# cwangrun/MGProto

Hardware: NVIDIA H100
Metric: images/sec (higher is better)
Workload: dtype f32

## Files before the change

mgproto_b200/csrc/abi.cu:

```cuda
#include "mgp_common.cuh"
#include <stdlib.h>
#include <string.h>

int mgp_logprob_simt_launch(const float* xhat, const float* mu, const float* sigma, float eps, float eps_log,
                            float* out, int layout, int B, int HW, int P, int D, float* ws, cudaStream_t st);
bool mgp_logprob_tc_supported(int layout, int B, int HW, int P, int D, int assume_iso);
size_t mgp_logprob_tc_ws_bytes(long long N, int P, int D);
int mgp_logprob_tc_launch(const float* xhat, const float* mu, const float* sigma, float eps, float eps_log,
                          float* out, int layout, int B, int HW, int P, int D, void* ws, size_t ws_bytes,
                          int reuse_operands, int assume_iso, int x_staged, cudaStream_t st);

extern "C" int mgp_abi_version(void) { return MGP_ABI_VERSION; }

extern "C" const char* mgp_error_string(int code) {
    switch (code) {
        case MGP_OK: return "ok";
        case MGP_ERR_INVALID: return "mgproto_b200: invalid argument (null pointer, non-positive size or misalignment)";
        case MGP_ERR_UNSUPPORTED: return "mgproto_b200: shape not supported by the sm_90a kernels";
        case MGP_ERR_WORKSPACE: return "mgproto_b200: workspace too small";
        default: break;
    }
    if (code > 0) return cudaGetErrorString((cudaError_t)code);
    return "mgproto_b200: unknown error";
}

int g_mgp_em_fused = -1;
int mgp_opt_em_fused() {
    if (g_mgp_em_fused < 0) g_mgp_em_fused = getenv("MGP_EM_UNFUSED") ? 0 : 1;
    return g_mgp_em_fused;
}
void mgp_em_tc_set_prof(void* p, int cls);
extern "C" int mgp_debug_set_ptr(const char* key, void* p, int arg) {
    if (!key) return MGP_ERR_INVALID;
#ifdef MGP_WITH_TC
    if (strcmp(key, "em_tc_prof") == 0) { mgp_em_tc_set_prof(p, arg); return MGP_OK; }
#endif
    return MGP_ERR_INVALID;
}
int g_mgp_tc_z = -1;
int mgp_opt_tc_z() {
    if (g_mgp_tc_z < 0) g_mgp_tc_z = getenv("MGP_TC_NO_Z") ? 0 : 1;
    return g_mgp_tc_z;
}
int g_mgp_em_tc = -1;
int mgp_opt_em_tc() {
    if (g_mgp_em_tc < 0) g_mgp_em_tc = getenv("MGP_EM_NO_TC") ? 0 : 1;
    return g_mgp_em_tc;
}
int g_mgp_em_pipe = -1;
int mgp_opt_em_pipe() {
    if (g_mgp_em_pipe < 0) g_mgp_em_pipe = getenv("MGP_EM_NO_PIPE") ? 0 : 1;
    return g_mgp_em_pipe;
}
extern "C" int mgp_set_option(const char* key, int value) {
    if (!key) return MGP_ERR_INVALID;
    if (strcmp(key, "em_pipe") == 0) {
        const int prev = mgp_opt_em_pipe();
        g_mgp_em_pipe = value ? 1 : 0;
        return prev;
    }
    if (strcmp(key, "tc_z") == 0) {
        const int prev = mgp_opt_tc_z();
        g_mgp_tc_z = value ? 1 : 0;
        return prev;
    }
    if (strcmp(key, "em_tc") == 0) {
        const int prev = mgp_opt_em_tc();
        g_mgp_em_tc = value ? 1 : 0;
        return prev;
    }
    if (strcmp(key, "em_fused") == 0) {
        const int prev = mgp_opt_em_fused();
        g_mgp_em_fused = value ? 1 : 0;
        return prev;
    }
    return MGP_ERR_INVALID;
}

extern "C" int mgp_has_tensor_core_path(void) {
#ifdef MGP_WITH_TC
    return 1;
#else
    return 0;
#endif
}

extern "C" size_t mgp_logprob_ws_bytes(int B, int HW, int P, int D, int math) {
    size_t simt = ((size_t)P * D + P) * sizeof(float);
#ifdef MGP_WITH_TC
    if (math != MGP_MATH_FP32 && mgp_logprob_tc_supported(0, B, HW, P, D, math == MGP_MATH_TC_ISO || math == MGP_MATH_TC_ISO_REUSE)) {
        size_t tc = mgp_logprob_tc_ws_bytes((long long)B * HW, P, D);
        return tc > simt ? tc : simt;
    }
#endif
    (void)math; (void)B; (void)HW;
    return simt;
}

bool mgp_logprob_tcz_supported(int P, int D);
extern "C" int mgp_logprob_ws_is_prototype_only(int out_layout, int P, int D, int math) {
#ifdef MGP_WITH_TC
    return (out_layout == MGP_OUT_LOGP_NP && (math == MGP_MATH_TC_ISO || math == MGP_MATH_TC_ISO_REUSE) && mgp_opt_tc_z() &&
            P > 0 && mgp_logprob_tcz_supported(P, D)) ? 1 : 0;
#else
    (void)out_layout; (void)P; (void)D; (void)math;
    return 0;
#endif
}

extern "C" int mgp_logprob_fwd(const float* xhat_nd, const float* mu, const float* sigma, float eps, float eps_log,
                               float* out, int out_layout, int B, int HW, int P, int D, int math, void* ws,
                               size_t ws_bytes, void* stream) {
    const int x_staged = (math & MGP_MATH_X_STAGED_ISO) ? 1 : ((math & MGP_MATH_X_STAGED) ? 2 : 0);
    math &= 0xff;
    if (!xhat_nd || !mu || !sigma || !out || !ws) return MGP_ERR_INVALID;
    if (B <= 0 || HW <= 0 || P <= 0 || D <= 0 || (D & 3)) return MGP_ERR_INVALID;
    if (out_layout < MGP_OUT_LOGP_NP || out_layout > MGP_OUT_TOP1_BP) return MGP_ERR_INVALID;
    if (!mgp_aligned16(xhat_nd) || !mgp_aligned16(mu) || !mgp_aligned16(sigma) || !mgp_aligned16(out) ||
        !mgp_aligned16(ws))
        return MGP_ERR_INVALID;
    if ((long long)B * HW > 0x7fffffffLL) return MGP_ERR_UNSUPPORTED;
    if (ws_bytes < mgp_logprob_ws_bytes(B, HW, P, D, math)) return MGP_ERR_WORKSPACE;
    cudaStream_t st = (cudaStream_t)stream;
#ifdef MGP_WITH_TC
    const bool iso_mode = (math == MGP_MATH_TC_ISO || math == MGP_MATH_TC_ISO_REUSE);
    if (math == MGP_MATH_TC || math == MGP_MATH_AUTO || math == MGP_MATH_TC_REUSE || iso_mode) {
        if (mgp_logprob_tc_supported(out_layout, B, HW, P, D, iso_mode))
            return mgp_logprob_tc_launch(xhat_nd, mu, sigma, eps, eps_log, out, out_layout, B, HW, P, D, ws, ws_bytes,
                                         math == MGP_MATH_TC_REUSE ? 2 : (math == MGP_MATH_TC_ISO_REUSE ? 1 : 0), iso_mode,
                                         x_staged, st);
        if (math != MGP_MATH_AUTO) return MGP_ERR_UNSUPPORTED;
    }
#else
    if (math == MGP_MATH_TC || math == MGP_MATH_TC_REUSE || math == MGP_MATH_TC_ISO || math == MGP_MATH_TC_ISO_REUSE)
        return MGP_ERR_UNSUPPORTED;
#endif
    if (out_layout == MGP_OUT_TOP1_BP) return MGP_ERR_UNSUPPORTED;
    return mgp_logprob_simt_launch(xhat_nd, mu, sigma, eps, eps_log, out, out_layout, B, HW, P, D,
                                   reinterpret_cast<float*>(ws), st);
}
```

mgproto_b200/csrc/head.cu:

```cuda
#include "mgp_common.cuh"
#include <type_traits>

namespace {

template <int R, int NR>
__device__ __forceinline__ void warp_topT(const float* const (&rows)[NR], int rs, int HW, int T, int lane,
                                          float (&out_v)[NR], int (&out_i)[NR]) {
    unsigned key[NR][R];
#pragma unroll
    for (int i = 0; i < NR; ++i) {
#pragma unroll
        for (int r = 0; r < R; ++r) {
            const int j = lane + 32 * r;
            key[i][r] = (j < HW) ? f2key(rows[i][(size_t)j * rs]) : 0u;
        }
        out_v[i] = 0.f;
        out_i[i] = 0;
    }
    for (int t = 0; t < T; ++t) {
#pragma unroll
        for (int i = 0; i < NR; ++i) {
            unsigned lm = key[i][0];
#pragma unroll
            for (int r = 1; r < R; ++r) lm = max(lm, key[i][r]);
// ... 248 lines not shown
        for (int i = threadIdx.x; i < K * D; i += NTHR) same = same && (s_ri[i] == s_ri[(i / D) * D]);
        const bool iso = __syncthreads_and(same ? 1 : 0) != 0;
        for (int k = warp; k < K; k += NTHR / 32) {
            float mm = 0.f;
            for (int d = lane; d < D; d += 32) mm = fmaf(s_mu[k * D + d], s_mu[k * D + d], mm);
            mm = warp_sum(mm);
            if (lane == 0) s_mm[k] = mm;
        }
        __syncthreads();
        const int KHh = (K + 1) / 2;
        for (int it = threadIdx.x; it < 2 * HW; it += NTHR) {
            const int n = it >> 1, kb = (it & 1) * KHh, ke = min(K, kb + KHh);
            const float4* xr = reinterpret_cast<const float4*>(xhat + ((size_t)b * HW + n) * D);
            for (int k0 = kb; k0 < ke; k0 += 5) {
                float q[5] = {0.f, 0.f, 0.f, 0.f, 0.f};
                float2 q2[5], xx2 = make_float2(0.f, 0.f);
#pragma unroll
                for (int i = 0; i < 5; ++i) q2[i] = make_float2(0.f, 0.f);
                for (int d0 = 0; d0 < D / 4; d0 += 8) {
                    float4 xv[8];
#pragma unroll
                    for (int u = 0; u < 8; ++u) xv[u] = (d0 + u < D / 4) ? __ldg(xr + d0 + u) : make_float4(0.f, 0.f, 0.f, 0.f);
                    if (iso) {
#pragma unroll
                        for (int u = 0; u < 8; ++u) {
                            if (d0 + u >= D / 4) break;
                            const float2 x01 = make_float2(xv[u].x, xv[u].y), x23 = make_float2(xv[u].z, xv[u].w);
                            xx2 = ffma2(x01, x01, xx2);
                            xx2 = ffma2(x23, x23, xx2);
#pragma unroll
                            for (int i = 0; i < 5; ++i) {
                                const int k = min(k0 + i, K - 1);
                                const float4 m = *reinterpret_cast<const float4*>(s_mu + k * D + 4 * (d0 + u));
                                q2[i] = ffma2(x01, make_float2(m.x, m.y), q2[i]);
                                q2[i] = ffma2(x23, make_float2(m.z, m.w), q2[i]);
                            }
                        }
                    } else {
#pragma unroll
                        for (int u = 0; u < 8; ++u) {
                            if (d0 + u >= D / 4) break;
#pragma unroll
                            for (int i = 0; i < 5; ++i) {
                                const int k = min(k0 + i, K - 1);
                                const float4 m = *reinterpret_cast<const float4*>(s_mu + k * D + 4 * (d0 + u));
                                const float4 r = *reinterpret_cast<const float4*>(s_ri + k * D + 4 * (d0 + u));
                                float t;
                                t = (xv[u].x - m.x) * r.x; q[i] = fmaf(t, t, q[i]);
                                t = (xv[u].y - m.y) * r.y; q[i] = fmaf(t, t, q[i]);
                                t = (xv[u].z - m.z) * r.z; q[i] = fmaf(t, t, q[i]);
                                t = (xv[u].w - m.w) * r.w; q[i] = fmaf(t, t, q[i]);
                            }
                        }
                    }
                }
                if (iso) {
                    const float xx = xx2.x + xx2.y;
#pragma unroll
                    for (int i = 0; i < 5; ++i) {
                        const int k = min(k0 + i, K - 1);
                        const float ri = s_ri[k * D];
                        q[i] = ri * ri * (xx - 2.0f * (q2[i].x + q2[i].y) + s_mm[k]);
                    }
                }
#pragma unroll
                for (int i = 0; i < 5; ++i)
                    if (k0 + i < ke) lp[(k0 + i) * HWp + n] = -s_ls[k0 + i] - 0.5f * q[i];
            }
        }
        __syncthreads();
        for (int k0 = warp * NR; k0 < K; k0 += (NTHR / 32) * NR) {
            const float* rows[NR];
#pragma unroll
            for (int i = 0; i < NR; ++i) rows[i] = lp + min(k0 + i, K - 1) * HWp;
            float v[NR];
            int ix[NR];
            if (R <= 8) warp_topT_sorted<(R <= 8 ? R : 1), NR>(rows, 1, HW, T, lane, v, ix);
            else warp_topT<R, NR>(rows, 1, HW, T, lane, v, ix);
#pragma unroll
            for (int i = 0; i < NR; ++i) {
                const int k = k0 + i;
                if (k < K && lane < T) {
                    const int p = (int)g * K + k;
                    const float e = expf(v[i]);
                    winT[k * T + lane] = e;
                    vals[((size_t)b * P + p) * T + lane] = e;
                    idx[((size_t)b * P + p) * T + lane] = ix[i];
                }
            }
        }
    }
    __syncthreads();
    for (int e = threadIdx.x; e < C * T; e += NTHR) {
        const int c = e / T, t = e - c * T;
        const bool own = gok && (long long)c == g;
        float s = 0.f;
        for (int k = 0; k < K; ++k) s = fmaf(s_wd[c * K + k], own ? winT[k * T + t] : win0[c * K + k], s);
        logits[((size_t)b * C + c) * T + t] = logf(s);
    }
}

__global__ void proto_weight_kernel(const float* __restrict__ mu, const float* __restrict__ sigma,
                                    float* __restrict__ w, float* __restrict__ wm, float* __restrict__ wsc,
                                    int* __restrict__ noniso, size_t n, int D) {
    size_t i = (size_t)blockIdx.x * blockDim.x + threadIdx.x;
    if (i < n) {
        const float s = sigma[i];
        const float ww = 1.0f / (s * s);
        w[i] = ww;
        wm[i] = ww * mu[i];
        const size_t p = i / D;
        if (i == p * D) wsc[p] = ww;
        if (s != sigma[p * D]) atomicOr(noniso, 1);
    }
}

constexpr int LCAP = 2304;

template <int VEC> struct LaneVec { float v[VEC]; };
template <int VEC>
__device__ __forceinline__ LaneVec<VEC> lv_ldg(const float* p) {
    LaneVec<VEC> r;
    if constexpr (VEC == 4) { const float4 t = __ldg(reinterpret_cast<const float4*>(p)); r.v[0] = t.x; r.v[1] = t.y; r.v[2] = t.z; r.v[3] = t.w; }
    else { const float2 t = __ldg(reinterpret_cast<const float2*>(p)); r.v[0] = t.x; r.v[1] = t.y; }
    return r;
}
template <int VEC>
__device__ __forceinline__ LaneVec<VEC> lv_ldcg(const float* p) {
    LaneVec<VEC> r;
    if constexpr (VEC == 4) { const float4 t = __ldcg(reinterpret_cast<const float4*>(p)); r.v[0] = t.x; r.v[1] = t.y; r.v[2] = t.z; r.v[3] = t.w; }
    else { const float2 t = __ldcg(reinterpret_cast<const float2*>(p)); r.v[0] = t.x; r.v[1] = t.y; }
    return r;
}
template <int VEC>
__device__ __forceinline__ LaneVec<VEC> lv_ld(const float* p) {
    LaneVec<VEC> r;
    if constexpr (VEC == 4) { const float4 t = *reinterpret_cast<const float4*>(p); r.v[0] = t.x; r.v[1] = t.y; r.v[2] = t.z; r.v[3] = t.w; }
    else { const float2 t = *reinterpret_cast<const float2*>(p); r.v[0] = t.x; r.v[1] = t.y; }
    return r;
}
template <int VEC>
__device__ __forceinline__ void lv_st(float* p, const LaneVec<VEC>& r) {
    if constexpr (VEC == 4) *reinterpret_cast<float4*>(p) = make_float4(r.v[0], r.v[1], r.v[2], r.v[3]);
    else *reinterpret_cast<float2*>(p) = make_float2(r.v[0], r.v[1]);
}
template <int VEC>
__device__ __forceinline__ LaneVec<VEC> lv_zero() {
    LaneVec<VEC> r;
#pragma unroll
    for (int i = 0; i < VEC; ++i) r.v[i] = 0.f;
    return r;
}

template <int VEC>
__global__ void __launch_bounds__(256, VEC == 4 ? 2 : 4)
head_bwd_kernel(const float* __restrict__ gl, const float* __restrict__ logits, const float* __restrict__ vals,
                const int32_t* __restrict__ idx, const float* __restrict__ weight, const int64_t* __restrict__ gt,
                const float* __restrict__ xhat, const float* __restrict__ w, const float* __restrict__ wm,
                const float* __restrict__ wsc, const int* __restrict__ noniso, float* __restrict__ g_xhat, int HW,
                int C, int K, int D, int T) {
    constexpr int DC = 32 * VEC;
    using LV = LaneVec<VEC>;
    extern __shared__ float smem[];
    const bool aniso = (*noniso != 0);
    unsigned* lkey = reinterpret_cast<unsigned*>(smem);
    float* lval = reinterpret_cast<float*>(lkey + LCAP);
    unsigned* skey = reinterpret_cast<unsigned*>(lval + LCAP);
    float* sval = reinterpret_cast<float*>(skey + LCAP);
    int* bins = reinterpret_cast<int*>(sval + LCAP);
    float* Qs = reinterpret_cast<float*>(bins + 8 * HW);
    float* qg = Qs + C;
    __shared__ int wcount[8];
    __shared__ int lcount;
    __shared__ __align__(16) float part[16 * DC];
    __shared__ float part2[16];
    __shared__ int prow[16];
    __shared__ int mrow[16], mcount;

    const int b = blockIdx.x;
    const int d0 = blockIdx.y * DC;
    const int dc = min(DC, D - d0);
    const int P = C * K;
    const int lane = threadIdx.x & 31, warp = threadIdx.x >> 5;
    const bool has_gt = (gt != nullptr);
    const long long g = has_gt ? (long long)gt[b] : -1;

    if (has_gt) {
        if (C * T <= 2 * LCAP) {
            float* qtmp = reinterpret_cast<float*>(skey);
            const size_t lo = (size_t)b * C * T;
            for (int i = threadIdx.x; i < C * T; i += 256) qtmp[i] = gl[lo + i] / expf(logits[lo + i]);
            __syncthreads();
            for (int c = threadIdx.x; c < C; c += 256) {
                float q = 0.f;
                for (int t = 0; t < T; ++t) q += qtmp[c * T + t];
                Qs[c] = q;
            }
            if (g >= 0 && g < C)
                for (int t = threadIdx.x; t < T; t += 256) qg[t] = qtmp[(int)g * T + t];
        } else {
            for (int c = threadIdx.x; c < C; c += 256) {
                const size_t lo = ((size_t)b * C + c) * T;
                float q = 0.f;
                for (int t = 0; t < T; ++t) q += gl[lo + t] / expf(logits[lo + t]);
                Qs[c] = q;
            }
            if (g >= 0 && g < C)
                for (int t = threadIdx.x; t < T; t += 256) {
                    const size_t lo = ((size_t)b * C + (size_t)g) * T;
                    qg[t] = gl[lo + t] / expf(logits[lo + t]);
                }
        }
    }
    if (threadIdx.x == 0) lcount = 0;
    __syncthreads();

    const bool gvalid = has_gt && g >= 0 && g < C;
    const int E = has_gt ? (P + (gvalid ? K * (T - 1) : 0)) : P * T;
    auto entry = [&](int e, float& a, unsigned& key) {
        a = 0.f;
        key = 0;
        if (e < E) {
            int p, t;
            float qv;
            if (has_gt) {
                if (e < P) {
                    p = e; t = 0;
                    const int c = p / K;
                    qv = ((long long)c == g) ? qg[0] : Qs[c];
                } else {
                    const int r = e - P;
                    const int k = r / (T - 1);
                    t = 1 + (r - k * (T - 1));
                    p = (int)g * K + k;
                    qv = qg[t];
                }
            } else {
                p = e / T; t = e - p * T;
                const size_t lo = ((size_t)b * C + p / K) * T + t;
                qv = gl[lo] / expf(logits[lo]);
            }
            const int c = p / K;
            const size_t vi = ((size_t)b * P + p) * T + t;
            a = qv * __ldg(weight + (size_t)c * P + p) * vals[vi];
            key = (unsigned)p * 1024u + (unsigned)idx[vi];
        }
    };
    float a_nx;
    unsigned key_nx;
    entry(threadIdx.x, a_nx, key_nx);
    for (int e0 = 0; e0 < E; e0 += 256) {
        const float a = a_nx;
        const unsigned key = key_nx;
        entry(e0 + 256 + threadIdx.x, a_nx, key_nx);
        const bool keep = (a != 0.f);
        const unsigned bal = __ballot_sync(0xffffffffu, keep);
        if (lane == 0) wcount[warp] = __popc(bal);
        __syncthreads();
        int base = lcount;
        for (int wv = 0; wv < warp; ++wv) base += wcount[wv];
        if (keep) {
            const int pos = base + __popc(bal & ((1u << lane) - 1u));
            lkey[pos] = key;
            lval[pos] = a;
        }
        __syncthreads();
        if (threadIdx.x == 0) {
            int tot = 0;
            for (int wv = 0; wv < 8; ++wv) tot += wcount[wv];
            lcount += tot;
        }
        __syncthreads();
        const int cnt = lcount;
        const bool last = (e0 + 256 >= E);
        if (cnt + 256 > LCAP || last) {
            int* whist = bins;
            for (int i = threadIdx.x; i < 8 * HW; i += 256) whist[i] = 0;
            __syncthreads();
            const int seg = (cnt + 7) / 8, sb = min(cnt, warp * seg), se = min(cnt, sb + seg);
            for (int i0 = sb; i0 < se; i0 += 32) {
                const int i = i0 + lane;
                const int n = (i < se) ? (int)(lkey[i] & 1023u) : (0x10000 + lane);
                const unsigned m = __match_any_sync(0xffffffffu, n);
                if (i < se && (m & ((1u << lane) - 1u)) == 0) whist[warp * HW + n] += __popc(m);
                __syncwarp();
            }
            __syncthreads();
            if (warp == 0) {
                int carry = 0;
                for (int r0 = 0; r0 < HW; r0 += 32) {
                    const int r = r0 + lane;
                    int tot = 0;
                    if (r < HW)
                        for (int wv = 0; wv < 8; ++wv) tot += whist[wv * HW + r];
                    int x = tot;
#pragma unroll
                    for (int o = 1; o < 32; o <<= 1) {
                        const int y = __shfl_up_sync(0xffffffffu, x, o);
                        if (lane >= o) x += y;
                    }
                    int start = carry + x - tot;
                    if (r < HW)
                        for (int wv = 0; wv < 8; ++wv) {
                            const int c = whist[wv * HW + r];
                            whist[wv * HW + r] = start;
                            start += c;
                        }
                    carry += __shfl_sync(0xffffffffu, x, 31);
                }
            }
            __syncthreads();
            for (int i0 = sb; i0 < se; i0 += 32) {
                const int i = i0 + lane;
                const unsigned kk = (i < se) ? lkey[i] : 0u;
                const int n = (i < se) ? (int)(kk & 1023u) : (0x10000 + lane);
                const unsigned m = __match_any_sync(0xffffffffu, n);
                if (i < se) {
                    const int pos = whist[warp * HW + n] + __popc(m & ((1u << lane) - 1u));
                    skey[pos] = kk;
                    sval[pos] = lval[i];
                }
                __syncwarp();
                if (i < se && (m & ((1u << lane) - 1u)) == 0) whist[warp * HW + n] += __popc(m);
                __syncwarp();
            }
            __syncthreads();
            if (threadIdx.x < 16) prow[threadIdx.x] = -1;
            __syncthreads();
            const int dl = VEC * lane;
            const bool dok2 = dl < dc;
            const int dle = dok2 ? dl : 0;
            const float* xcol2 = xhat + (size_t)b * HW * D + d0 + dle;
            float* gcol = g_xhat + (size_t)b * HW * D + d0 + dle;
            {
                const int wseg = (cnt + 7) / 8, wb = min(cnt, warp * wseg), we = min(cnt, wb + wseg);
                const float* wmcol_l = wm + d0 + dle;
                const float* wcol_l = w + d0 + dle;
                int cur_n = -1;
                bool first_run = true;
                LV s1 = lv_zero<VEC>(), s2v = lv_zero<VEC>(), xpre = lv_zero<VEC>(), gpre = lv_zero<VEC>();
                float s2 = 0.f;
                auto flush = [&](int slot) {
                    if (slot < 0) {
                        LV v = gpre;
#pragma unroll
                        for (int i = 0; i < VEC; ++i) v.v[i] += aniso ? fmaf(-xpre.v[i], s2v.v[i], s1.v[i]) : fmaf(-xpre.v[i], s2, s1.v[i]);
                        if (dok2) lv_st<VEC>(gcol + (size_t)cur_n * D, v);
                    } else {
                        LV v = s1;
                        if (aniso) {
#pragma unroll
                            for (int i = 0; i < VEC; ++i) v.v[i] = fmaf(-xpre.v[i], s2v.v[i], v.v[i]);
                        }
                        if (dok2) lv_st<VEC>(part + (warp * 2 + slot) * DC + dl, v);
                        if (lane == 0) { part2[warp * 2 + slot] = aniso ? 0.f : s2; prow[warp * 2 + slot] = cur_n; }
                    }
                };
                auto walk = [&](auto aniso_tag) {
                    constexpr bool AN = decltype(aniso_tag)::value;
                    constexpr int PF = (VEC == 4 && !AN) ? 16 : 8;
                    for (int i0 = wb; i0 < we; i0 += 32) {
                        const int i = i0 + lane;
                        const bool ok = i < we;
                        const unsigned kk = skey[ok ? i : we - 1];
                        const float av = ok ? sval[i] : 0.f;
                        const float v2 = (!AN && ok) ? av * __ldg(wsc + (kk >> 10)) : 0.f;
                        const int m = min(32, we - i0);
                        for (int j0 = 0; j0 < m; j0 += PF) {
                            LV fm[PF], fw[AN ? PF : 1];
#pragma unroll
                            for (int u = 0; u < PF; ++u) {
                                const unsigned ku = __shfl_sync(0xffffffffu, kk, j0 + u);
                                const unsigned po = (ku >> 10) * (unsigned)D;
                                fm[u] = lv_ldg<VEC>(wmcol_l + po);
                                if constexpr (AN) fw[u] = lv_ldg<VEC>(wcol_l + po);
                            }
#pragma unroll
                            for (int u = 0; u < PF; ++u) {
                                const int n = (int)(__shfl_sync(0xffffffffu, kk, j0 + u) & 1023u);
                                const float a = __shfl_sync(0xffffffffu, av, j0 + u);
                                if (n != cur_n) {
                                    if (cur_n >= 0) {
                                        flush(first_run ? 0 : -1);
                                        first_run = false;
                                    }
                                    cur_n = n;
                                    xpre = lv_ldg<VEC>(xcol2 + (size_t)n * D);
                                    gpre = lv_ldcg<VEC>(gcol + (size_t)n * D);
                                    s1 = lv_zero<VEC>();
                                    s2v = lv_zero<VEC>();
                                    s2 = 0.f;
                                }
#pragma unroll
                                for (int i = 0; i < VEC; ++i) s1.v[i] = fmaf(a, fm[u].v[i], s1.v[i]);
                                if constexpr (AN) {
#pragma unroll
                                    for (int i = 0; i < VEC; ++i) s2v.v[i] = fmaf(a, fw[u].v[i], s2v.v[i]);
                                } else {
                                    s2 += __shfl_sync(0xffffffffu, v2, j0 + u);
                                }
                            }
                        }
                    }
                };
                if (aniso) walk(std::true_type{}); else walk(std::false_type{});
                if (cur_n >= 0) flush(first_run ? 0 : 1);
            }
            __syncthreads();
            if (warp == 0) {
                int j = -1, last = -1;
                LV acc = lv_zero<VEC>();
                float a2 = 0.f;
                for (int i = 0; i < 16; ++i) {
                    const int n = prow[i];
                    if (n < 0) continue;
                    const LV v = lv_ld<VEC>(part + i * DC + dl);
                    const float p2 = part2[i];
                    __syncwarp();
                    if (n != last) { ++j; last = n; acc = lv_zero<VEC>(); a2 = 0.f; }
#pragma unroll
                    for (int q = 0; q < VEC; ++q) acc.v[q] += v.v[q];
                    a2 += p2;
                    lv_st<VEC>(part + j * DC + dl, acc);
                    if (lane == 0) { part2[j] = a2; mrow[j] = n; }
                    __syncwarp();
                }
                if (lane == 0) mcount = j + 1;
            }
            __syncthreads();
            for (int j = warp; j < mcount; j += 8) {
                const int n = mrow[j];
                const LV xv = lv_ldg<VEC>(xcol2 + (size_t)n * D);
                LV gv = lv_ldcg<VEC>(gcol + (size_t)n * D);
                const LV v = lv_ld<VEC>(part + j * DC + dl);
                const float p2 = part2[j];
#pragma unroll
                for (int q = 0; q < VEC; ++q) gv.v[q] += fmaf(-xv.v[q], p2, v.v[q]);
                if (dok2) lv_st<VEC>(gcol + (size_t)n * D, gv);
            }
            __syncthreads();
            if (threadIdx.x == 0) lcount = 0;
            __syncthreads();
        }
    }
}

__global__ void __launch_bounds__(256)
mine_ce_kernel(const float* __restrict__ out, const int64_t* __restrict__ gt, float* __restrict__ loss_b,
               float* __restrict__ grad, int B, int C, int T, float mine_coef) {
    extern __shared__ float sm[];
    float* lse = sm;
    const int b = blockIdx.x;
    const int lane = threadIdx.x & 31, warp = threadIdx.x >> 5;
    const float* ob = out + (size_t)b * C * T;
    for (int t = warp; t < T; t += 8) {
        float m = -INFINITY;
        for (int c = lane; c < C; c += 32) m = fmaxf(m, ob[(size_t)c * T + t]);
        m = warp_max(m);
        float se = 0.f;
        for (int c = lane; c < C; c += 32) se += expf(ob[(size_t)c * T + t] - m);
        se = warp_sum(se);
        if (lane == 0) lse[t] = m + logf(se);
    }
    __syncthreads();
    const long long g = gt[b];
    const float wt0 = 1.0f / (float)B, wtm = (T > 1) ? mine_coef / ((float)(T - 1) * (float)B) : 0.f;
    if (threadIdx.x == 0) {
        float l = 0.f;
        for (int t = 0; t < T; ++t) l += (t == 0 ? wt0 : wtm) * (lse[t] - ob[(size_t)g * T + t]);
        loss_b[b] = l;
    }
    float* gb = grad + (size_t)b * C * T;
    for (int i = threadIdx.x; i < C * T; i += 256) {
        const int c = i / T, t = i - c * T;
        const float wv = (t == 0) ? wt0 : wtm;
        gb[i] = wv * (expf(ob[i] - lse[t]) - (((long long)c == g) ? 1.0f : 0.0f));
    }
}

__global__ void push_argmin_kernel(const float* __restrict__ logp, const int64_t* __restrict__ labels,
                                   int32_t* __restrict__ arg, float* __restrict__ val, int HW, int C, int K, int B) {
    const int wg = blockIdx.x * (blockDim.x >> 5) + (threadIdx.x >> 5);
    const int lane = threadIdx.x & 31;
    if (wg >= B * K) return;
    const int b = wg / K, k = wg - b * K;
    const long long c = labels[b];
    if (c < 0 || c >= C) {
        if (lane == 0) { arg[wg] = -1; val[wg] = 0.f; }
        return;
    }
    const float* row = logp + ((size_t)b * C * K + (size_t)c * K + k) * HW;
    unsigned best = 0;
    int bi = 0x7fffffff;
    for (int i = lane; i < HW; i += 32) {
        unsigned kk = f2key(row[i]);
        if (kk > best) { best = kk; bi = i; }
    }
    const unsigned wb = __reduce_max_sync(0xffffffffu, best);
    const int wi = __reduce_min_sync(0xffffffffu, (best == wb) ? bi : 0x7fffffff);
    if (lane == 0) {
        arg[wg] = wi;
        val[wg] = -expf(key2f(wb));
    }
}

__global__ void push_from_top1_kernel(const unsigned long long* __restrict__ best, const int64_t* __restrict__ labels,
                                      int32_t* __restrict__ arg, float* __restrict__ val, int B, int C, int K) {
    const int i = blockIdx.x * blockDim.x + threadIdx.x;
    if (i >= B * K) return;
    const int b = i / K, k = i - b * K;
    const long long c = labels[b];
    if (c < 0 || c >= C) { arg[i] = -1; val[i] = 0.f; return; }
    const unsigned long long pk = best[(size_t)b * C * K + (size_t)c * K + k];
    arg[i] = (int)(0xffffffffu - (unsigned)(pk & 0xffffffffull));
    val[i] = -expf(key2f((unsigned)(pk >> 32)));
}

}

static int head_select_launch(const float* logp, int from_np, const float* weight_cp, const int64_t* gt, float* logits,
                              float* vals, int32_t* idx, int B, int HW, int C, int K, int T, void* stream,
                              int is_prob = 0) {
    if (!logp || !vals || !idx || (!is_prob && (!weight_cp || !logits))) return MGP_ERR_INVALID;
    if (B <= 0 || HW <= 0 || C <= 0 || K <= 0 || T <= 0) return MGP_ERR_INVALID;
    if (T > 32 || T > HW || HW > 1024) return MGP_ERR_UNSUPPORTED;
    int CT = 64 / K;
    if (CT < 1) CT = 1;
    if (CT > C) CT = C;
    size_t smem = (size_t)CT * K * T * sizeof(float);
    if (from_np) smem += (size_t)HW * (CT * K + 1) * sizeof(float);
    if (smem > 200 * 1024) return MGP_ERR_UNSUPPORTED;
    dim3 grid((C + CT - 1) / CT, B);
    cudaStream_t st = (cudaStream_t)stream;
    const int R = (HW + 31) / 32;
#define MGP_LAUNCH_SEL2(RR, NRR, NP)                                                                                 \
    do {                                                                                                             \
        MGP_CUDA(cudaFuncSetAttribute(head_select_kernel<RR, NRR, NP>, cudaFuncAttributeMaxDynamicSharedMemorySize,  \
                                      (int)smem));                                                                   \
        MGP_CUDA(cudaFuncSetAttribute(head_select_kernel<RR, NRR, NP>,                                               \
                                      cudaFuncAttributePreferredSharedMemoryCarveout, NP ? 100 : 25));               \
        head_select_kernel<RR, NRR, NP><<<grid, 256, smem, st>>>(logp, weight_cp, gt, logits, vals, idx, HW, C, K,   \
                                                                 T, CT, is_prob);                                    \
    } while (0)
#define MGP_LAUNCH_SEL(RR, NRR)                                                                                      \
    do {                                                                                                             \
        if (from_np) MGP_LAUNCH_SEL2(RR, NRR, true);                                                                 \
        else MGP_LAUNCH_SEL2(RR, NRR, false);                                                                        \
    } while (0)
    if (R <= 2) MGP_LAUNCH_SEL(2, 4);
    else if (R <= 4) MGP_LAUNCH_SEL(4, 4);
    else if (R <= 7) MGP_LAUNCH_SEL(7, 4);
    else if (R <= 13) MGP_LAUNCH_SEL(13, 2);
    else if (R <= 25) MGP_LAUNCH_SEL(25, 1);
    else MGP_LAUNCH_SEL(32, 1);
#undef MGP_LAUNCH_SEL
#undef MGP_LAUNCH_SEL2
    MGP_CHECK_LAUNCH();
    return MGP_OK;
}

extern "C" int mgp_head_select(const float* logp_bphw, const float* weight_cp, const int64_t* gt, float* logits,
                               float* vals, int32_t* idx, int B, int HW, int C, int K, int T, void* stream) {
    return head_select_launch(logp_bphw, 0, weight_cp, gt, logits, vals, idx, B, HW, C, K, T, stream);
}

extern "C" int mgp_head_select_np(const float* logp_np, const float* weight_cp, const int64_t* gt, float* logits,
                                  float* vals, int32_t* idx, int B, int HW, int C, int K, int T, void* stream) {
    return head_select_launch(logp_np, 1, weight_cp, gt, logits, vals, idx, B, HW, C, K, T, stream);
}

namespace {
__global__ void topt_gather_kernel(const float* __restrict__ x, const int32_t* __restrict__ idx, float* __restrict__ feats,
                                   int HW, int P, int D, int T) {
    const int b = blockIdx.y, p = blockIdx.x;
    __shared__ int s_i[32];
    if (threadIdx.x < T) s_i[threadIdx.x] = idx[((size_t)b * P + p) * T + threadIdx.x];
    __syncthreads();
    float* dst = feats + ((size_t)b * P + p) * D * T;
    const float* src = x + (size_t)b * D * HW;
    for (int e = threadIdx.x; e < D * T; e += blockDim.x) {
        const int d = e / T, t = e - d * T;
        dst[e] = src[(size_t)d * HW + s_i[t]];
    }
}
}

namespace {
__global__ void ood_score_kernel(const float* __restrict__ out0, int stride_b, int stride_c, float* __restrict__ p_sum,
                                 float* __restrict__ p_mean, int64_t* __restrict__ pred, int B, int C) {
    const int b = blockIdx.x * (blockDim.x >> 5) + (threadIdx.x >> 5);
    const int lane = threadIdx.x & 31;
    if (b >= B) return;
    float s = 0.f, best = -INFINITY;
    int bi = 0x7fffffff;
    for (int c = lane; c < C; c += 32) {
        const float v = out0[(size_t)b * stride_b + (size_t)c * stride_c];
        s += expf(v);
        if (v > best) { best = v; bi = c; }
    }
    s = warp_sum(s);
#pragma unroll
    for (int o = 16; o > 0; o >>= 1) {
        const float ov = __shfl_xor_sync(0xffffffffu, best, o);
        const int oi = __shfl_xor_sync(0xffffffffu, bi, o);
        if (ov > best || (ov == best && oi < bi)) { best = ov; bi = oi; }
    }
    if (lane == 0) {
        p_sum[b] = s;
        p_mean[b] = s / (float)C;
        pred[b] = bi;
    }
}
}

extern "C" int mgp_ood_score(const float* out0, int stride_b, int stride_c, float* p_sum, float* p_mean, int64_t* pred,
                             int B, int C, void* stream) {
    if (!out0 || !p_sum || !p_mean || !pred || B <= 0 || C <= 0 || stride_b <= 0 || stride_c <= 0) return MGP_ERR_INVALID;
    ood_score_kernel<<<(B + 7) / 8, 256, 0, (cudaStream_t)stream>>>(out0, stride_b, stride_c, p_sum, p_mean, pred, B, C);
    MGP_CHECK_LAUNCH();
    return MGP_OK;
}

extern "C" int mgp_topt_pool(const float* sims_bphw, const float* x_nchw, float* vals, int32_t* idx, float* feats, int B,
                             int HW, int C, int K, int D, int T, void* stream) {
    if (!sims_bphw || !vals || !idx || (feats && !x_nchw) || D <= 0) return MGP_ERR_INVALID;
    int rc = head_select_launch(sims_bphw, 0, nullptr, nullptr, nullptr, vals, idx, B, HW, C, K, T, stream, 1);
    if (rc != MGP_OK || !feats) return rc;
    dim3 grid(C * K, B);
    topt_gather_kernel<<<grid, 128, 0, (cudaStream_t)stream>>>(x_nchw, idx, feats, HW, C * K, D, T);
    MGP_CHECK_LAUNCH();
    return MGP_OK;
}

extern "C" int mgp_head_select_top1(const uint64_t* best, const float* xhat_nd, const float* mu, const float* sigma,
                                    const float* weight_cp, const int64_t* gt, float* logits, float* vals, int32_t* idx,
                                    int B, int HW, int C, int K, int D, int T, void* stream) {
    if (!best || !xhat_nd || !mu || !sigma || !weight_cp || !gt || !logits || !vals || !idx) return MGP_ERR_INVALID;
    if (B <= 0 || HW <= 0 || C <= 0 || K <= 0 || D <= 0 || T <= 0 || (D & 3)) return MGP_ERR_INVALID;
    if (T > 32 || T > HW || HW > 1024) return MGP_ERR_UNSUPPORTED;
    const int P = C * K;
    const size_t smem = ((size_t)2 * P + (size_t)K * T + (size_t)K * (HW + 1) + (size_t)2 * K * D + 2 * K + 4) * sizeof(float);
    if (smem > 200 * 1024) return MGP_ERR_UNSUPPORTED;
    const int R = (HW + 31) / 32;
    cudaStream_t st = (cudaStream_t)stream;
#define MGP_LAUNCH_T1(RR, NRR)                                                                                       \
    do {                                                                                                             \
        MGP_CUDA(cudaFuncSetAttribute(head_top1_kernel<RR, NRR, 256>, cudaFuncAttributeMaxDynamicSharedMemorySize,   \
                                      (int)smem));                                                                   \
        head_top1_kernel<RR, NRR, 256><<<B, 256, smem, st>>>(reinterpret_cast<const unsigned long long*>(best),      \
                                                             xhat_nd, mu, sigma, weight_cp, gt, logits, vals, idx,   \
                                                             HW, C, K, D, T);                                         \
    } while (0)
    if (R <= 4) MGP_LAUNCH_T1(4, 2);
    else if (R <= 7) MGP_LAUNCH_T1(7, 2);
    else if (R <= 13) MGP_LAUNCH_T1(13, 1);
    else if (R <= 25) MGP_LAUNCH_T1(25, 1);
    else MGP_LAUNCH_T1(32, 1);
#undef MGP_LAUNCH_T1
    MGP_CHECK_LAUNCH();
    return MGP_OK;
}

extern "C" size_t mgp_head_bwd_ws_bytes(int B, int HW, int P, int D) {
    return ((size_t)2 * P * D + (size_t)B * HW * D + (size_t)P + 64) * sizeof(float);
}

extern "C" int mgp_head_bwd(const float* grad_logits, const float* logits, const float* vals, const int32_t* idx,
                            const float* weight_cp, const int64_t* gt, const float* xhat_nd, const float* inv_norm,
                            const float* mu, const float* sigma, void* ws, size_t ws_bytes, float* g_x_nchw, int B,
                            int HW, int C, int K, int D, int T, void* stream) {
    if (!grad_logits || !logits || !vals || !idx || !weight_cp || !xhat_nd || !inv_norm || !mu || !sigma || !ws ||
        !g_x_nchw)
        return MGP_ERR_INVALID;
    if (B <= 0 || HW <= 0 || C <= 0 || K <= 0 || D <= 0 || T <= 0) return MGP_ERR_INVALID;
    if (HW > 1024 || (size_t)C * K >= (1u << 22)) return MGP_ERR_UNSUPPORTED;
    const int P = C * K;
    if (ws_bytes < mgp_head_bwd_ws_bytes(B, HW, P, D)) return MGP_ERR_WORKSPACE;
    cudaStream_t st = (cudaStream_t)stream;
    float* w = reinterpret_cast<float*>(ws);
    float* wm = w + (size_t)P * D;
    float* g_xhat = wm + (size_t)P * D;
    float* wsc = g_xhat + (size_t)B * HW * D;
    int* noniso = reinterpret_cast<int*>(wsc + P);
    const size_t npd = (size_t)P * D;
    MGP_CUDA(cudaMemsetAsync(noniso, 0, sizeof(int), st));
    proto_weight_kernel<<<(unsigned)((npd + 255) / 256), 256, 0, st>>>(mu, sigma, w, wm, wsc, noniso, npd, D);
    MGP_CHECK_LAUNCH();
    static const bool vec2_forced = getenv("MGP_HEAD_BWD_VEC2") != nullptr;
    const int DC = ((D % 128) == 0 && !vec2_forced) ? 128 : 64;
    size_t smem = (size_t)LCAP * 16 + (size_t)(8 * HW + C + T) * 4;
    if (smem > 200 * 1024) return MGP_ERR_UNSUPPORTED;
    MGP_CUDA(cudaFuncSetAttribute(head_bwd_kernel<2>, cudaFuncAttributeMaxDynamicSharedMemorySize, (int)smem));
    MGP_CUDA(cudaFuncSetAttribute(head_bwd_kernel<4>, cudaFuncAttributeMaxDynamicSharedMemorySize, (int)smem));
    MGP_CUDA(cudaMemsetAsync(g_xhat, 0, (size_t)B * HW * D * sizeof(float), st));
    dim3 grid(B, (D + DC - 1) / DC);
    if (DC == 128)
        head_bwd_kernel<4><<<grid, 256, smem, st>>>(grad_logits, logits, vals, idx, weight_cp, gt, xhat_nd, w, wm, wsc, noniso,
                                                    g_xhat, HW, C, K, D, T);
    else
        head_bwd_kernel<2><<<grid, 256, smem, st>>>(grad_logits, logits, vals, idx, weight_cp, gt, xhat_nd, w, wm, wsc, noniso,
                                                    g_xhat, HW, C, K, D, T);
    MGP_CHECK_LAUNCH();
    return mgp_normalize_bwd(g_xhat, xhat_nd, inv_norm, g_x_nchw, B, D, HW, stream);
}

extern "C" int mgp_mine_ce(const float* out, const int64_t* gt, float* loss_b, float* grad, int B, int C, int T,
                           float mine_coef, void* stream) {
    if (!out || !gt || !loss_b || !grad || B <= 0 || C <= 0 || T <= 0) return MGP_ERR_INVALID;
    mine_ce_kernel<<<B, 256, (size_t)T * sizeof(float), (cudaStream_t)stream>>>(out, gt, loss_b, grad, B, C, T, mine_coef);
    MGP_CHECK_LAUNCH();
    return MGP_OK;
}

extern "C" int mgp_push_argmin(const float* logp_bphw, const int64_t* labels, int32_t* arg, float* val, int B, int HW,
                               int C, int K, void* stream) {
    if (!logp_bphw || !labels || !arg || !val || B <= 0 || HW <= 0 || C <= 0 || K <= 0) return MGP_ERR_INVALID;
    const int warps = B * K;
    push_argmin_kernel<<<(warps + 7) / 8, 256, 0, (cudaStream_t)stream>>>(logp_bphw, labels, arg, val, HW, C, K, B);
    MGP_CHECK_LAUNCH();
    return MGP_OK;
}

extern "C" int mgp_push_argmin_top1(const unsigned long long* best_bp, const int64_t* labels, int32_t* arg, float* val, int B,
                                    int C, int K, void* stream) {
    if (!best_bp || !labels || !arg || !val || B <= 0 || C <= 0 || K <= 0) return MGP_ERR_INVALID;
    push_from_top1_kernel<<<(B * K + 255) / 256, 256, 0, (cudaStream_t)stream>>>(best_bp, labels, arg, val, B, C, K);
    MGP_CHECK_LAUNCH();
    return MGP_OK;
}
```

mgproto_b200/ops.py:

```python
from __future__ import annotations

import collections
import os

import torch

from . import _lib
from ._lib import (MGP_MATH_AUTO, MGP_MATH_FP32, MGP_MATH_TC, MGP_MATH_TC_ISO, MGP_MATH_TC_ISO_REUSE, MGP_MATH_TC_REUSE,
                   MGP_MATH_X_STAGED, MGP_MATH_X_STAGED_ISO,
                   MGP_OUT_LOGP_BPHW,
                   MGP_OUT_LOGP_NP, MGP_OUT_NEGP_BPHW, MGP_OUT_TOP1_BP, check)

__all__ = ["normalize_fwd", "logprob", "logprob_top1", "head_select", "head_select_top1", "head_level0", "head_forward", "HeadFunction", "mined_gather", "bank_enqueue",
           "bank_linearize", "bank_shadow_sync", "em_plan", "em_stats", "em_update", "update_gmm", "em_estep", "em_mstep_closed", "em_mstep_div", "topt_pool", "ood_score", "push_argmin", "push_argmin_top1", "mine_cross_entropy",
           "MATH_MODES"]

MATH_MODES = {"fp32": MGP_MATH_FP32, "tc": MGP_MATH_TC, "auto": MGP_MATH_AUTO, "tc_reuse": MGP_MATH_TC_REUSE,
              "tc_iso": MGP_MATH_TC_ISO, "tc_iso_reuse": MGP_MATH_TC_ISO_REUSE}

_iso_cache = {}


_PROTO_OPERANDS = collections.OrderedDict()


def sigma_is_isotropic(sigma: torch.Tensor) -> bool:
    key = (sigma.data_ptr(), sigma._version, sigma.numel(), sigma.shape[-1], str(sigma.device))
    hit = _iso_cache.get(key)
    if hit is None:
        hit = bool((sigma == sigma[..., :1]).all().item())
        if len(_iso_cache) >= 8:
            _iso_cache.clear()
        _iso_cache[key] = hit
    return hit

_launches = 0


def launch_count() -> int:
    return _launches


def _count(n: int):
    global _launches
    _launches += n


_op_device = None
_CHECK_ALL = os.environ.get("MGP_CHECK_DEVICES", "0") == "1"


_raw_stream = getattr(torch._C, "_cuda_getCurrentRawStream", None)


def _stream() -> int:
    if _raw_stream is not None and _op_device is not None and _op_device.index is not None:
        return _raw_stream(_op_device.index)
    return torch.cuda.current_stream(_op_device).cuda_stream


class _on_device:

    def __init__(self, fn):
        self.fn = fn
        self.__name__ = getattr(fn, "__name__", "op")
        self.__doc__ = fn.__doc__

    def __call__(self, *args, **kw):
        global _op_device
        t0 = args[0] if args else None
        dev = t0.device if isinstance(t0, torch.Tensor) else None
        if dev is not None and not _CHECK_ALL and dev.type == "cuda" and dev.index == torch.cuda.current_device():
            prev, _op_device = _op_device, dev
            try:
                return self.fn(*args, **kw)
            finally:
                _op_device = prev
        dev = None
        for a in list(args) + list(kw.values()):
            if isinstance(a, (tuple, list)):
                cand = [t for t in a if isinstance(t, torch.Tensor)]
            else:
                cand = [a] if isinstance(a, torch.Tensor) else []
            for t in cand:
                if t.is_cuda:
                    if dev is None:
                        dev = t.device
                    elif t.device != dev:
                        raise RuntimeError("mgproto_b200: %s got tensors on %s and %s" % (self.__name__, dev, t.device))
        prev = _op_device
        if dev is None or dev.index == torch.cuda.current_device():
            _op_device = dev
            try:
                return self.fn(*args, **kw)
            finally:
                _op_device = prev
        with torch.cuda.device(dev):
            _op_device = dev
            try:
                return self.fn(*args, **kw)
            finally:
                _op_device = prev


def _req(t: torch.Tensor, dtype, name: str) -> torch.Tensor:
    if not isinstance(t, torch.Tensor) or not t.is_cuda:
        raise RuntimeError("mgproto_b200: %s must be a CUDA tensor (there is no CPU path)" % name)
    if t.dtype != dtype:
        raise RuntimeError("mgproto_b200: %s must be %s, got %s" % (name, dtype, t.dtype))
    if not t.is_contiguous():
        raise RuntimeError("mgproto_b200: %s must be contiguous" % name)
    return t


def _p(t):
    return 0 if t is None else t.data_ptr()


def _math(math) -> int:
    return MATH_MODES[math] if isinstance(math, str) else int(math)


@_on_device
def normalize_fwd(x_bdhw: torch.Tensor, want_nchw: bool = False, stage=None):
    x = _req(x_bdhw, torch.float32, "x")
    B, D, H, W = x.shape
    HW = H * W
    xhat = torch.empty((B * HW, D), device=x.device, dtype=torch.float32)
    inv = torch.empty((B * HW,), device=x.device, dtype=torch.float32)
    nchw = torch.empty_like(x) if want_nchw else None
    lib = _lib.load()
    if stage is not None:
        P, aniso = stage
        nbytes = lib.mgp_logprob_ws_bytes(B, HW, int(P), D, MGP_MATH_TC)
        ws = torch.empty((max(16, nbytes),), device=x.device, dtype=torch.uint8)
        check(lib.mgp_normalize_fwd_stage(x.data_ptr(), xhat.data_ptr(), inv.data_ptr(), _p(nchw), ws.data_ptr(), nbytes,
                                          B, D, HW, int(P), 1 if aniso else 0, _stream()), "mgp_normalize_fwd_stage")
        _count(1)
        return xhat, inv, nchw, ws
    check(lib.mgp_normalize_fwd(x.data_ptr(), xhat.data_ptr(), inv.data_ptr(), _p(nchw), B, D, HW, _stream()),
          "mgp_normalize_fwd")
    _count(1)
    return xhat, inv, nchw


def _stage_for_top1(B, HW, P, D, sg, math):
    m = _math(math)
    if m not in (MGP_MATH_AUTO, MGP_MATH_TC, MGP_MATH_TC_ISO) or D not in (64, 128) or HW < 32 or HW > 256:
        return None
    if not _lib.load().mgp_has_tensor_core_path():
        return None
    return (P, not sigma_is_isotropic(sg))


@_on_device
def logprob(xhat_nd, mu_pd, sigma_pd, layout=MGP_OUT_LOGP_NP, B=None, HW=None, eps=0.0, eps_log=0.0,
            math="auto", ws=None, out=None, return_ws=False):
    x = _req(xhat_nd, torch.float32, "xhat")
    mu = _req(mu_pd, torch.float32, "mu")
    sg = _req(sigma_pd, torch.float32, "sigma")
    N, D = x.shape
    P = mu.shape[0]
    if mu.shape != (P, D) or sg.shape != (P, D):
        raise RuntimeError("mgproto_b200: mu/sigma must be [P, D]")
    if layout == MGP_OUT_LOGP_NP:
        B_, HW_ = N, 1
        shape = (N, P)
    else:
        if B is None or HW is None or B * HW != N:
            raise RuntimeError("mgproto_b200: BPHW layouts need B*HW == N")
        B_, HW_ = B, HW
        shape = (B, P, HW)
    if out is None:
        out = torch.empty(shape, device=x.device, dtype=torch.float32)
    elif tuple(out.shape) != shape:
        raise RuntimeError("mgproto_b200: out has the wrong shape")
    lib = _lib.load()
    m = _math(math)
    if m == MGP_MATH_AUTO:
        iso = sigma_is_isotropic(sg)
        if D > 128:
            m = MGP_MATH_TC_ISO if (D == 256 and iso) else MGP_MATH_FP32
        elif iso and D in (64, 128):
            m = MGP_MATH_TC_ISO
    nbytes = lib.mgp_logprob_ws_bytes(B_, HW_, P, D, m)
    cache_key = None
    if ws is None and m == MGP_MATH_TC_ISO and lib.mgp_logprob_ws_is_prototype_only(int(layout), P, D, m):
# ... 464 lines not shown
```

Before: 407,500.

## Fuse normalize backward and NCHW transpose into head backward kernel

When D is 128 and labels are present, the head backward kernel now applies the normalization backward (projection against xhat and scaling by inv_norm) per row in a warp epilogue. It then transposes the result to NCHW in shared memory, zero-filling rows that were never touched according to a per-CTA bitmask. This removes the memset of g_xhat, the read-modify-write of g_xhat, and the separate normalize-backward launch. It adds shared-memory transposes and syncs inside the kernel. The iso cache change also keeps a reference to sigma so the cached data pointer cannot be reused by a different tensor.

```diff
diff --git a/mgproto_b200/csrc/abi.cu b/mgproto_b200/csrc/abi.cu
--- a/mgproto_b200/csrc/abi.cu
+++ b/mgproto_b200/csrc/abi.cu
@@ -52,8 +52,15 @@
     if (g_mgp_em_pipe < 0) g_mgp_em_pipe = getenv("MGP_EM_NO_PIPE") ? 0 : 1;
     return g_mgp_em_pipe;
 }
+int g_mgp_head_bwd_fused = 1;
+int mgp_opt_head_bwd_fused() { return g_mgp_head_bwd_fused; }
 extern "C" int mgp_set_option(const char* key, int value) {
     if (!key) return MGP_ERR_INVALID;
+    if (strcmp(key, "head_bwd_fused") == 0) {
+        const int prev = g_mgp_head_bwd_fused;
+        g_mgp_head_bwd_fused = value ? 1 : 0;
+        return prev;
+    }
     if (strcmp(key, "em_pipe") == 0) {
         const int prev = mgp_opt_em_pipe();
         g_mgp_em_pipe = value ? 1 : 0;
diff --git a/mgproto_b200/csrc/head.cu b/mgproto_b200/csrc/head.cu
--- a/mgproto_b200/csrc/head.cu
+++ b/mgproto_b200/csrc/head.cu
@@ -424,13 +424,14 @@
     return r;
 }
 
-template <int VEC>
+template <int VEC, bool FUSED>
 __global__ void __launch_bounds__(256, VEC == 4 ? 2 : 4)
 head_bwd_kernel(const float* __restrict__ gl, const float* __restrict__ logits, const float* __restrict__ vals,
                 const int32_t* __restrict__ idx, const float* __restrict__ weight, const int64_t* __restrict__ gt,
                 const float* __restrict__ xhat, const float* __restrict__ w, const float* __restrict__ wm,
-                const float* __restrict__ wsc, const int* __restrict__ noniso, float* __restrict__ g_xhat, int HW,
-                int C, int K, int D, int T) {
+                const float* __restrict__ wsc, const int* __restrict__ noniso, float* __restrict__ g_xhat,
+                const float* __restrict__ inv_norm, float* __restrict__ gx, int HW, int C, int K, int D, int T) {
+    static_assert(!FUSED || VEC == 4, "the fused epilogue needs a whole 128-dim row per CTA");
     constexpr int DC = 32 * VEC;
     using LV = LaneVec<VEC>;
     extern __shared__ float smem[];
@@ -442,6 +443,7 @@
     int* bins = reinterpret_cast<int*>(sval + LCAP);
     float* Qs = reinterpret_cast<float*>(bins + 8 * HW);
     float* qg = Qs + C;
+    __shared__ unsigned rowbits[32];
     __shared__ int wcount[8];
     __shared__ int lcount;
     __shared__ __align__(16) float part[16 * DC];
@@ -457,6 +459,7 @@
     const bool has_gt = (gt != nullptr);
     const long long g = has_gt ? (long long)gt[b] : -1;
 
+    if (FUSED && threadIdx.x < 32) rowbits[threadIdx.x] = 0u;
     if (has_gt) {
         if (C * T <= 2 * LCAP) {
             float* qtmp = reinterpret_cast<float*>(skey);
@@ -604,6 +607,25 @@
             const int dle = dok2 ? dl : 0;
             const float* xcol2 = xhat + (size_t)b * HW * D + d0 + dle;
             float* gcol = g_xhat + (size_t)b * HW * D + d0 + dle;
+            auto finish = [&](int n, const LV& gv, const LV& xv, float inv) {
+                float* rb = reinterpret_cast<float*>(lkey) + warp * 256;
+                __syncwarp();
+                lv_st<VEC>(rb + dl, gv);
+                lv_st<VEC>(rb + 128 + dl, xv);
+                __syncwarp();
+                float gq[4], xq[4], dot = 0.f;
+#pragma unroll
+                for (int q = 0; q < 4; ++q) {
+                    gq[q] = rb[lane + 32 * q];
+                    xq[q] = rb[128 + lane + 32 * q];
+                    dot = fmaf(gq[q], xq[q], dot);
+                }
+                dot = warp_sum(dot);
+                float* row = g_xhat + ((size_t)b * HW + n) * D;
+#pragma unroll
+                for (int q = 0; q < 4; ++q) row[lane + 32 * q] = fmaf(-xq[q], dot, gq[q]) * inv;
+                if (lane == 0) atomicOr(&rowbits[n >> 5], 1u << (n & 31));
+            };
             {
                 const int wseg = (cnt + 7) / 8, wb = min(cnt, warp * wseg), we = min(cnt, wb + wseg);
                 const float* wmcol_l = wm + d0 + dle;
@@ -611,13 +633,14 @@
                 int cur_n = -1;
                 bool first_run = true;
                 LV s1 = lv_zero<VEC>(), s2v = lv_zero<VEC>(), xpre = lv_zero<VEC>(), gpre = lv_zero<VEC>();
-                float s2 = 0.f;
+                float s2 = 0.f, invpre = 0.f;
                 auto flush = [&](int slot) {
                     if (slot < 0) {
                         LV v = gpre;
 #pragma unroll
                         for (int i = 0; i < VEC; ++i) v.v[i] += aniso ? fmaf(-xpre.v[i], s2v.v[i], s1.v[i]) : fmaf(-xpre.v[i], s2, s1.v[i]);
-                        if (dok2) lv_st<VEC>(gcol + (size_t)cur_n * D, v);
+                        if constexpr (FUSED) finish(cur_n, v, xpre, invpre);
+                        else if (dok2) lv_st<VEC>(gcol + (size_t)cur_n * D, v);
                     } else {
                         LV v = s1;
                         if (aniso) {
@@ -658,7 +681,8 @@
                                     }
                                     cur_n = n;
                                     xpre = lv_ldg<VEC>(xcol2 + (size_t)n * D);
-                                    gpre = lv_ldcg<VEC>(gcol + (size_t)n * D);
+                                    if constexpr (FUSED) invpre = __ldg(inv_norm + (size_t)b * HW + n);
+                                    else gpre = lv_ldcg<VEC>(gcol + (size_t)n * D);
                                     s1 = lv_zero<VEC>();
                                     s2v = lv_zero<VEC>();
                                     s2 = 0.f;
@@ -703,12 +727,33 @@
             for (int j = warp; j < mcount; j += 8) {
                 const int n = mrow[j];
                 const LV xv = lv_ldg<VEC>(xcol2 + (size_t)n * D);
-                LV gv = lv_ldcg<VEC>(gcol + (size_t)n * D);
+                LV gv = FUSED ? lv_zero<VEC>() : lv_ldcg<VEC>(gcol + (size_t)n * D);
                 const LV v = lv_ld<VEC>(part + j * DC + dl);
                 const float p2 = part2[j];
 #pragma unroll
                 for (int q = 0; q < VEC; ++q) gv.v[q] += fmaf(-xv.v[q], p2, v.v[q]);
-                if (dok2) lv_st<VEC>(gcol + (size_t)n * D, gv);
+                if constexpr (FUSED) finish(n, gv, xv, __ldg(inv_norm + (size_t)b * HW + n));
+                else if (dok2) lv_st<VEC>(gcol + (size_t)n * D, gv);
+            }
+            if constexpr (FUSED) {
+                __syncthreads();
+                float* tile = reinterpret_cast<float*>(lkey);
+                const float* gb = g_xhat + (size_t)b * HW * D;
+                float* ob = gx + (size_t)b * D * HW;
+                for (int hw0 = 0; hw0 < HW; hw0 += 32) {
+                    for (int r = warp; r < 32 && hw0 + r < HW; r += 8) {
+                        const int n = hw0 + r;
+                        const bool has = (rowbits[n >> 5] >> (n & 31)) & 1u;
+#pragma unroll
+                        for (int q = 0; q < 4; ++q)
+                            tile[(lane + 32 * q) * 33 + r] = has ? __ldcg(gb + (size_t)n * D + lane + 32 * q) : 0.f;
+                    }
+                    __syncthreads();
+                    const int hw = hw0 + lane;
+                    if (hw < HW)
+                        for (int d = warp; d < 128; d += 8) ob[(size_t)d * HW + hw] = tile[d * 33 + lane];
+                    __syncthreads();
+                }
             }
             __syncthreads();
             if (threadIdx.x == 0) lcount = 0;
@@ -933,6 +978,8 @@
     return MGP_OK;
 }
 
+int mgp_opt_head_bwd_fused();
+
 extern "C" size_t mgp_head_bwd_ws_bytes(int B, int HW, int P, int D) {
     return ((size_t)2 * P * D + (size_t)B * HW * D + (size_t)P + 64) * sizeof(float);
 }
@@ -962,16 +1009,26 @@
     const int DC = ((D % 128) == 0 && !vec2_forced) ? 128 : 64;
     size_t smem = (size_t)LCAP * 16 + (size_t)(8 * HW + C + T) * 4;
     if (smem > 200 * 1024) return MGP_ERR_UNSUPPORTED;
-    MGP_CUDA(cudaFuncSetAttribute(head_bwd_kernel<2>, cudaFuncAttributeMaxDynamicSharedMemorySize, (int)smem));
-    MGP_CUDA(cudaFuncSetAttribute(head_bwd_kernel<4>, cudaFuncAttributeMaxDynamicSharedMemorySize, (int)smem));
+    MGP_CUDA(cudaFuncSetAttribute(head_bwd_kernel<2, false>, cudaFuncAttributeMaxDynamicSharedMemorySize, (int)smem));
+    MGP_CUDA(cudaFuncSetAttribute(head_bwd_kernel<4, false>, cudaFuncAttributeMaxDynamicSharedMemorySize, (int)smem));
+    dim3 grid(B, (D + DC - 1) / DC);
+    const long long e_max = (long long)P + (long long)K * (T - 1);
+    const bool fused = DC == 128 && D == 128 && gt != nullptr && mgp_opt_head_bwd_fused() &&
+                       256 * ((e_max + 255) / 256) <= LCAP;
+    if (fused) {
+        MGP_CUDA(cudaFuncSetAttribute(head_bwd_kernel<4, true>, cudaFuncAttributeMaxDynamicSharedMemorySize, (int)smem));
+        head_bwd_kernel<4, true><<<grid, 256, smem, st>>>(grad_logits, logits, vals, idx, weight_cp, gt, xhat_nd, w, wm, wsc,
+                                                          noniso, g_xhat, inv_norm, g_x_nchw, HW, C, K, D, T);
+        MGP_CHECK_LAUNCH();
+        return MGP_OK;
+    }
     MGP_CUDA(cudaMemsetAsync(g_xhat, 0, (size_t)B * HW * D * sizeof(float), st));
-    dim3 grid(B, (D + DC - 1) / DC);
     if (DC == 128)
-        head_bwd_kernel<4><<<grid, 256, smem, st>>>(grad_logits, logits, vals, idx, weight_cp, gt, xhat_nd, w, wm, wsc, noniso,
-                                                    g_xhat, HW, C, K, D, T);
+        head_bwd_kernel<4, false><<<grid, 256, smem, st>>>(grad_logits, logits, vals, idx, weight_cp, gt, xhat_nd, w, wm, wsc,
+                                                           noniso, g_xhat, nullptr, nullptr, HW, C, K, D, T);
     else
-        head_bwd_kernel<2><<<grid, 256, smem, st>>>(grad_logits, logits, vals, idx, weight_cp, gt, xhat_nd, w, wm, wsc, noniso,
-                                                    g_xhat, HW, C, K, D, T);
+        head_bwd_kernel<2, false><<<grid, 256, smem, st>>>(grad_logits, logits, vals, idx, weight_cp, gt, xhat_nd, w, wm, wsc,
+                                                           noniso, g_xhat, nullptr, nullptr, HW, C, K, D, T);
     MGP_CHECK_LAUNCH();
     return mgp_normalize_bwd(g_xhat, xhat_nd, inv_norm, g_x_nchw, B, D, HW, stream);
 }
diff --git a/mgproto_b200/ops.py b/mgproto_b200/ops.py
--- a/mgproto_b200/ops.py
+++ b/mgproto_b200/ops.py
@@ -28,11 +28,11 @@
     key = (sigma.data_ptr(), sigma._version, sigma.numel(), sigma.shape[-1], str(sigma.device))
     hit = _iso_cache.get(key)
     if hit is None:
-        hit = bool((sigma == sigma[..., :1]).all().item())
+        hit = (bool((sigma == sigma[..., :1]).all().item()), sigma)
         if len(_iso_cache) >= 8:
             _iso_cache.clear()
         _iso_cache[key] = hit
-    return hit
+    return hit[0]
 
 _launches = 0
 
```

After: 419,600 (median of 6 runs). 3.0% higher.
